# trailofbits/reverie

Measured on AMD Instinct MI355X. Metric: prover AND-gates/sec on GF(2) Bristol circuit; 1/2/4/8-GPU; proof bit-exact, higher is better.
Workload: dtype u32; 1 GPU; synthetic layered AND/XOR GF(2) circuit, 10027008 gates (5014185 AND), 4096 inputs, 153 layers x 65536, p_and=0.5, 256 reps x 8 players, 40 online; parallelism=reps/1, levels=163, compile_hint=RV_COMPILE_WHOLE_PROVER, gate_stream_bytes=334698564

## Files before the change

reverie_amd/csrc/interp.hip:

```cpp
#include <stdlib.h>

#include <algorithm>

#include "gf2dev.h"
#include "internal.h"
#include "launch.h"

namespace rv {

static size_t g_device_lds_limit = 160 * 1024;
void set_device_lds_limit(size_t bytes) { g_device_lds_limit = bytes; }
size_t device_lds_limit() { return g_device_lds_limit; }


__device__ __forceinline__ uint32_t gather_rows(const uint32_t* rows, const uint32_t* ids, uint32_t NQ, uint32_t q) {
    uint32_t v = 0;
#pragma unroll
    for (int i = 0; i < RV_LIN_K; i++) v ^= rows[(size_t)ids[i] * NQ + q];
    return v;
}
__device__ __forceinline__ uint32_t gather_corr_byte(const uint8_t* corr, const uint32_t* ids, uint32_t NQ, uint32_t o) {
    uint32_t v = 0;
#pragma unroll
    for (int i = 0; i < RV_LIN_K; i++) v ^= corr[(size_t)ids[i] * (NQ >> 1) + o];
    return v;
}
__device__ __forceinline__ uint32_t gather_corr(const uint8_t* corr, const uint32_t* ids, uint32_t NQ, uint32_t q) {
    return (gather_corr_byte(corr, ids, NQ, q >> 1) >> (4 * (q & 1))) & 0xFu;
}

__device__ __forceinline__ uint32_t gather_vclr(const uint8_t* vclr, const uint32_t* ids) {
    uint32_t v = 0;
#pragma unroll
    for (int i = 0; i < RV_LIN_K; i++) v ^= vclr[ids[i]];
    return v;
}

__device__ __forceinline__ uint32_t vc_nib(uint64_t c, uint32_t q) {
    const uint32_t w = (q & 8) ? (uint32_t)(c >> 32) : (uint32_t)c;
    return q < 16 ? (w >> (4 * (q & 7))) & 0xFu : 0u;
}
__device__ __forceinline__ uint64_t gather_vc(const uint64_t* vc, const uint32_t* ids) {
    uint64_t v = 0;
#pragma unroll
    for (int i = 0; i < RV_LIN_K; i++) v ^= vc[ids[i]];
    return v;
}
__device__ __forceinline__ void vc_store(uint64_t* vc, size_t row, uint32_t q, uint32_t smeared) {
    uint32_t v = q < 16 ? compress4(smeared) << (4 * (q & 7)) : 0u;
    v |= (uint32_t)__builtin_amdgcn_update_dpp(0, (int)v, 0x111, 0xF, 0xF, true);
    v |= (uint32_t)__builtin_amdgcn_update_dpp(0, (int)v, 0x112, 0xF, 0xF, true);
    v |= (uint32_t)__builtin_amdgcn_update_dpp(0, (int)v, 0x114, 0xF, 0xF, true);
    if (q == 7 || q == 15) ((uint32_t*)(vc + row))[q >> 3] = v;
}
constexpr bool is_verify(int mode) { return mode == MODE_VERIFY || mode == MODE_VERIFY_C; }

template <int MODE>
__device__ __forceinline__ void interp_one(const Gate& g, const InterpParams& p, uint32_t NQ, uint32_t q, uint32_t onm) {
    switch (g_op(g)) {
    case G_INPUT: {
        const uint32_t lam = p.rows[(size_t)g.m * NQ + q];
        uint32_t corr;
        if (!is_verify(MODE)) {
            const uint32_t w = p.wit[g.x] ? 0xFFFFFFFFu : 0u;
            corr = w ^ recon32(lam);
        } else {
            corr = onm ? (p.sup_in[(size_t)g.x * p.sup_nq + q] & onm) : 0u;
        }
        if (!is_verify(MODE) || onm) p.on[(size_t)g.eo * NQ + q] = corr;
        if (MODE == MODE_PROVE_V) {
            if (q == 0) p.vclr[g.dst] = p.wit[g.x] ? 1 : 0;
        } else if (MODE == MODE_VERIFY_C) {
            vc_store(p.vc, g.dst, q, corr);
        } else {
            store_bits(p.corr, g.dst, NQ, q, corr);
        }
        break;
    }
    case G_XORK: {
        p.rows[(size_t)g.dst * NQ + q] = gather_rows(p.rows, g.a, NQ, q) ^ gather_rows(p.rows, g.b, NQ, q);
        if (MODE == MODE_PROVE_V) {
            if (q == 0) p.vclr[g.dst] = (uint8_t)((g_ca(g) ^ gather_vclr(p.vclr, g.a) ^ gather_vclr(p.vclr, g.b)) & 1u);
            break;
        }
        if (MODE == MODE_VERIFY_C) {
            if (q == 0) p.vc[g.dst] = gather_vc(p.vc, g.a) ^ gather_vc(p.vc, g.b) ^ (g_ca(g) ? ~0ull : 0ull);
            break;
        }
        if (!(q & 1)) {
            const size_t h = NQ >> 1, o = q >> 1;
            const uint32_t c = (g_ca(g) ? 0xFFu : 0u) ^ gather_corr_byte(p.corr, g.a, NQ, o) ^ gather_corr_byte(p.corr, g.b, NQ, o);
            p.corr[(size_t)g.dst * h + o] = (uint8_t)c;
        }
        break;
    }
    case G_RANDOM: {
        if (MODE == MODE_VERIFY_C) {
            if (q == 0) p.vc[g.dst] = 0;
            break;
        }
        if (!(q & 1)) p.corr[(size_t)g.dst * (NQ >> 1) + (q >> 1)] = 0;
        break;
    }
    case G_MUL: {
        const uint32_t lx = gather_rows(p.rows, g.a, NQ, q), ly = gather_rows(p.rows, g.b, NQ, q);
        const uint32_t lab = p.rows[(size_t)g.m * NQ + q], lnew = p.rows[(size_t)(g.m + 1) * NQ + q];
        const uint32_t a = recon32(lx), b = recon32(ly), c = recon32(lab);
        uint32_t cx, cy, vx = 0, vy = 0;
        if (MODE == MODE_PROVE_V) {
            vx = (gather_vclr(p.vclr, g.a) ^ g_ca(g)) & 1u;
            vy = (gather_vclr(p.vclr, g.b) ^ g_cb(g)) & 1u;
            cx = a ^ (vx ? 0xFFFFFFFFu : 0u);
            cy = b ^ (vy ? 0xFFFFFFFFu : 0u);
        } else if (MODE == MODE_VERIFY_C) {
            cx = expand4(vc_nib(gather_vc(p.vc, g.a), q)) ^ (g_ca(g) ? 0xFFFFFFFFu : 0u);
            cy = expand4(vc_nib(gather_vc(p.vc, g.b), q)) ^ (g_cb(g) ? 0xFFFFFFFFu : 0u);
        } else {
            cx = expand4(gather_corr(p.corr, g.a, NQ, q)) ^ (g_ca(g) ? 0xFFFFFFFFu : 0u);
            cy = expand4(gather_corr(p.corr, g.b, NQ, q)) ^ (g_cb(g) ? 0xFFFFFFFFu : 0u);
        }
        uint32_t delta = (a & b) ^ c;
        uint32_t s = (ly & cx) ^ (lx & cy) ^ lab ^ lnew;
        uint32_t r;
        if (!is_verify(MODE)) {
            r = recon32(s);
        } else {
            if (onm) {
                delta = (p.sup_corr[(size_t)g.ep * p.sup_nq + q] & onm) | (delta & ~onm);
                s ^= p.sup_rec[(size_t)g.x * p.sup_nq + q];
            }
            r = recon32(s) & onm;
        }
        if (!is_verify(MODE) || onm) p.on[(size_t)g.eo * NQ + q] = s;
        store_bits(p.pre, g.ep, NQ, q, delta);
        if (MODE == MODE_PROVE_V) {
            if (q == 0) p.vclr[g.dst] = (uint8_t)(vx & vy);
        } else if (MODE == MODE_VERIFY_C) {
            vc_store(p.vc, g.dst, q, r ^ delta ^ (cx & cy));
        } else {
            store_bits(p.corr, g.dst, NQ, q, r ^ delta ^ (cx & cy));
        }
        break;
    }
    case G_RECON: {
        uint32_t m = gather_rows(p.rows, g.a, NQ, q);
        if (is_verify(MODE) && onm) m ^= p.sup_rec[(size_t)g.x * p.sup_nq + q];
        if (MODE == MODE_PROVE || onm) p.on[(size_t)g.eo * NQ + q] = m;
        uint32_t r = recon32(m);
        if (is_verify(MODE)) r &= onm;
        const uint32_t cx = expand4(gather_corr(p.corr, g.a, NQ, q)) ^ (g_ca(g) ? 0xFFFFFFFFu : 0u);
        p.rows[(size_t)g.dst * NQ + q] = 0;
        store_bits(p.corr, g.dst, NQ, q, r ^ cx);
        break;
    }
    case G_ASSERT: {
        uint32_t m = gather_rows(p.rows, g.a, NQ, q);
        if (is_verify(MODE) && onm) m ^= p.sup_rec[(size_t)g.x * p.sup_nq + q];
        if (!is_verify(MODE) || onm) p.on[(size_t)g.eo * NQ + q] = m;
        if (MODE == MODE_PROVE_V) {
            if (q == 0 && ((gather_vclr(p.vclr, g.a) ^ g_ca(g)) & 1u) != 0) atomicOr(p.err, RV_E_WITNESS_INVALID);
        } else {
            const uint32_t cx = expand4(MODE == MODE_VERIFY_C ? vc_nib(gather_vc(p.vc, g.a), q) : gather_corr(p.corr, g.a, NQ, q)) ^ (g_ca(g) ? 0xFFFFFFFFu : 0u);
            if (MODE == MODE_PROVE) {
                if ((recon32(m) ^ cx) != 0) atomicOr(p.err, RV_E_WITNESS_INVALID);
            } else {
                if (((recon32(m) ^ cx) & onm) != 0) atomicOr(p.err, RV_DEV_ZERO_CHECK);
            }
        }
        break;
    }
    default:
        break;
    }
}

template <int MODE>
__global__ __launch_bounds__(256) void k_interp(const Gate* __restrict__ gates, uint32_t lo, uint32_t hi, InterpParams p) {
    const uint32_t NQ = p.NQ;
    const uint32_t tid = blockIdx.x * blockDim.x + threadIdx.x;
    const uint32_t q = tid % NQ;
    const uint32_t worker = tid / NQ;
    const uint32_t n_workers = (gridDim.x * blockDim.x) / NQ;
    const uint32_t onm = (is_verify(MODE)) ? p.on_mask[q] : 0u;
    for (uint32_t gi = lo + worker; gi < hi; gi += n_workers) {
        const Gate g = gates[gi];
        interp_one<MODE>(g, p, NQ, q, onm);
    }
}

#ifndef RV_INTERP_UNROLL
#define RV_INTERP_UNROLL 4
#endif
#ifndef RV_INTERP_UNROLL_SMALL
#define RV_INTERP_UNROLL_SMALL 2
#endif
#ifndef RV_INTERP_UNROLL_MID
#define RV_INTERP_UNROLL_MID 4
#endif
#ifndef RV_INTERP_UNROLL_FAST
#define RV_INTERP_UNROLL_FAST 4
#endif
#ifndef RV_INTERP_UXOR_FAST
#define RV_INTERP_UXOR_FAST 0
#endif
__host__ __device__ constexpr int interp_unroll(int NQ, bool general = true) {
    return NQ >= 64 ? (general ? RV_INTERP_UNROLL : RV_INTERP_UNROLL_FAST) : NQ >= 32 ? RV_INTERP_UNROLL_MID : RV_INTERP_UNROLL_SMALL;
}

struct PfPlan {
    uint32_t dist;
    uint32_t rem;
    uint32_t n[2][4];
    uint32_t start[2][4];
};
template <uint32_t STEP>
__device__ __forceinline__ const Gate* pf_target(const Gate* __restrict__ gates, const PfPlan& pf, uint32_t t) {
    uint32_t tt = t + pf.dist;
#pragma unroll
    for (int k = 0; k < 2; k++) {
#pragma unroll
        for (int c = 0; c < 4; c++) {
            if (tt < pf.n[k][c]) return gates + pf.start[k][c] + tt * STEP;
            tt -= pf.n[k][c];
        }
        tt += pf.rem;
    }
    return nullptr;
}
template <uint32_t STEP>
__device__ __forceinline__ uint32_t pf_touch(const Gate* g, uint32_t lane) {
    constexpr uint32_t BYTES = STEP * (uint32_t)sizeof(Gate), NL = (BYTES + 127) / 128;
    uint32_t v = 0;
    if (g && lane <= NL) v = *(const uint32_t*)((const char*)g + (lane < NL ? lane * 128 : BYTES - 4));
    return v;
}
__device__ __forceinline__ void pf_sink(uint32_t v) { asm volatile("" ::"v"(v)); }

template <int MODE, int NQ, int U, int KA, int KB>
__device__ __forceinline__ void mulU(const Gate* __restrict__ gates, uint32_t g0, const InterpParams& p, uint32_t sub, uint32_t q,
                                     uint32_t onm, const Gate* pf = nullptr) {
    constexpr uint32_t GPW = 64 / NQ, H = NQ / 2;
    const bool on_wr = !is_verify(MODE) || ((__ballot(onm != 0) >> ((sub * NQ + q) & ~7u)) & 0xFFull) != 0;
    Gate g[U];
#pragma unroll
    for (int u = 0; u < U; u++) g[u] = gates[g0 + u * GPW + sub];
    uint32_t lx[U], ly[U], lab[U], lnew[U], bx[U], by[U], sc[U], sr[U];
    uint32_t ra[U][KA], ca[U][KA], rb[U][KB], cb[U][KB];
    const uint32_t* const vc32 = (const uint32_t*)p.vc + ((q >> 3) & 1u);
#pragma unroll
    for (int u = 0; u < U; u++) {
        const int na = (int)g_na(g[u]), nb = (int)g_nb(g[u]);
#pragma unroll
        for (int i = 0; i < KA; i++) {
            ra[u][i] = 0;
            ca[u][i] = 0;
            if (i == 0 || i < na) {
                ra[u][i] = p.rows[(size_t)g[u].a[i] * NQ + q];
                ca[u][i] = MODE == MODE_VERIFY_C ? vc32[2 * (size_t)g[u].a[i]]
                                                 : MODE == MODE_PROVE_V ? p.vclr[g[u].a[i]] : p.corr[(size_t)g[u].a[i] * H + (q >> 1)];
            }
        }
#pragma unroll
        for (int i = 0; i < KB; i++) {
            rb[u][i] = 0;
            cb[u][i] = 0;
            if (i == 0 || i < nb) {
                rb[u][i] = p.rows[(size_t)g[u].b[i] * NQ + q];
                cb[u][i] = MODE == MODE_VERIFY_C ? vc32[2 * (size_t)g[u].b[i]]
                                                 : MODE == MODE_PROVE_V ? p.vclr[g[u].b[i]] : p.corr[(size_t)g[u].b[i] * H + (q >> 1)];
            }
        }
        lab[u] = __builtin_nontemporal_load(&p.rows[(size_t)g[u].m * NQ + q]);
        lnew[u] = p.rows[(size_t)(g[u].m + 1) * NQ + q];
        if (is_verify(MODE)) {
            sc[u] = sr[u] = 0;
            if (onm) {
                sc[u] = p.sup_corr[(size_t)g[u].ep * p.sup_nq + q];
                sr[u] = p.sup_rec[(size_t)g[u].x * p.sup_nq + q];
            }
        }
    }
    const uint32_t pfv = pf_touch<U * GPW>(pf, sub * NQ + q);
#pragma unroll
    for (int u = 0; u < U; u++) {
        lx[u] = ra[u][0];
        bx[u] = ca[u][0];
        ly[u] = rb[u][0];
        by[u] = cb[u][0];
#pragma unroll
        for (int i = 1; i < KA; i++) {
            lx[u] ^= ra[u][i];
            bx[u] ^= ca[u][i];
        }
#pragma unroll
        for (int i = 1; i < KB; i++) {
            ly[u] ^= rb[u][i];
            by[u] ^= cb[u][i];
        }
    }
#pragma unroll
    for (int u = 0; u < U; u++) {
        const uint32_t a = recon32(lx[u]), b = recon32(ly[u]), c = recon32(lab[u]);
        uint32_t cx, cy;
        const uint32_t vx = (bx[u] ^ g_ca(g[u])) & 1u, vy = (by[u] ^ g_cb(g[u])) & 1u;
        if (MODE == MODE_PROVE_V) {
            cx = a ^ (vx ? 0xFFFFFFFFu : 0u);
            cy = b ^ (vy ? 0xFFFFFFFFu : 0u);
        } else if (MODE == MODE_VERIFY_C) {
            cx = expand4(q < 16 ? (bx[u] >> (4 * (q & 7))) & 0xFu : 0u) ^ (g_ca(g[u]) ? 0xFFFFFFFFu : 0u);
            cy = expand4(q < 16 ? (by[u] >> (4 * (q & 7))) & 0xFu : 0u) ^ (g_cb(g[u]) ? 0xFFFFFFFFu : 0u);
        } else {
            cx = expand4((bx[u] >> (4 * (q & 1))) & 0xFu) ^ (g_ca(g[u]) ? 0xFFFFFFFFu : 0u);
            cy = expand4((by[u] >> (4 * (q & 1))) & 0xFu) ^ (g_cb(g[u]) ? 0xFFFFFFFFu : 0u);
        }
        uint32_t delta = (a & b) ^ c;
        uint32_t s = (ly[u] & cx) ^ (lx[u] & cy) ^ lab[u] ^ lnew[u];
        uint32_t r = 0;
        if (MODE == MODE_PROVE) {
            r = recon32(s);
        } else if (is_verify(MODE)) {
            delta = (sc[u] & onm) | (delta & ~onm);
            s ^= sr[u];
            r = recon32(s) & onm;
        }
        if (!is_verify(MODE) || on_wr) __builtin_nontemporal_store(s, &p.on[(size_t)g[u].eo * NQ + q]);
        store_bits(p.pre, g[u].ep, NQ, q, delta);
        if (MODE == MODE_PROVE_V) {
            if (q == 0) p.vclr[g[u].dst] = (uint8_t)(vx & vy);
        } else if (MODE == MODE_VERIFY_C) {
            vc_store(p.vc, g[u].dst, q, r ^ delta ^ (cx & cy));
        } else {
            store_bits(p.corr, g[u].dst, NQ, q, r ^ delta ^ (cx & cy));
        }
    }
    pf_sink(pfv);
}

template <int MODE, int NQ, int U, int N>
__device__ __forceinline__ void xorU(const Gate* __restrict__ gates, uint32_t g0, const InterpParams& p, uint32_t sub, uint32_t q,
                                     const Gate* pf = nullptr) {
    constexpr uint32_t GPW = 64 / NQ, H = NQ / 2;
    Gate g[U];
#pragma unroll
    for (int u = 0; u < U; u++) g[u] = gates[g0 + u * GPW + sub];
    uint32_t x[U], bx[U], rr[U][N], cc[U][N];
#pragma unroll
    for (int u = 0; u < U; u++) {
        const int na = (int)g_na(g[u]), nb = (int)g_nb(g[u]);
#pragma unroll
        for (int i = 0; i < N; i++) {
            const uint32_t id = (N == 2) ? g[u].a[i] : (i < RV_LIN_K ? g[u].a[i] : g[u].b[i - RV_LIN_K]);
            rr[u][i] = 0;
            cc[u][i] = 0;
            if (N == 2 || (i < RV_LIN_K ? i < na : i - RV_LIN_K < nb)) {
                rr[u][i] = p.rows[(size_t)id * NQ + q];
                if (MODE == MODE_PROVE_V) {
                    if (q == 0) cc[u][i] = p.vclr[id];
                } else if (MODE == MODE_VERIFY_C) {
                    if (q < 2) cc[u][i] = ((const uint32_t*)p.vc)[2 * (size_t)id + q];
                } else if (q < H) {
                    cc[u][i] = p.corr[(size_t)id * H + q];
                }
            }
        }
    }
    const uint32_t pfv = pf_touch<U * GPW>(pf, sub * NQ + q);
#pragma unroll
    for (int u = 0; u < U; u++) {
        x[u] = 0;
        bx[u] = 0;
#pragma unroll
        for (int i = 0; i < N; i++) {
            x[u] ^= rr[u][i];
            bx[u] ^= cc[u][i];
        }
    }
#pragma unroll
    for (int u = 0; u < U; u++) {
        p.rows[(size_t)g[u].dst * NQ + q] = x[u];
        if (MODE == MODE_PROVE_V) {
            if (q == 0) p.vclr[g[u].dst] = (uint8_t)((bx[u] ^ g_ca(g[u])) & 1u);
        } else if (MODE == MODE_VERIFY_C) {
            if (q < 2) ((uint32_t*)p.vc)[2 * (size_t)g[u].dst + q] = bx[u] ^ (g_ca(g[u]) ? 0xFFFFFFFFu : 0u);
        } else if (q < H) {
            p.corr[(size_t)g[u].dst * H + q] = (uint8_t)(bx[u] ^ (g_ca(g[u]) ? 0xFFu : 0u));
        }
    }
    pf_sink(pfv);
}

template <int MODE, int NQ, bool GENERAL = true, bool PF = false, int UXOR = 0>
__device__ __forceinline__ void run_level(const Gate* __restrict__ gates, const LevelRange& r, const InterpParams& p, uint32_t wave,
                                          uint32_t n_waves, uint32_t lane, uint32_t onm, const Gate* pf_gates = nullptr,
                                          const PfPlan* pf = nullptr) {
    constexpr uint32_t GPW = 64 / NQ;
    const uint32_t q = lane % NQ, sub = lane / NQ;
    constexpr int U = interp_unroll(NQ, GENERAL);
    constexpr int UX = UXOR ? UXOR : U;
    static_assert(!PF || UX == U, "the prefetch plan assumes one step size");
    uint32_t slot = 0;
    auto my = [&](uint32_t used) { return (wave + n_waves - used % n_waves) % n_waves; };
    const uint32_t begin[5] = {r.lo, r.mul11, r.mul, r.xor2, r.xork}, end[5] = {r.mul11, r.mul, r.xor2, r.xork, r.hi};
    uint32_t rest[5];
#pragma unroll
    for (int c = 0; c < 4; c++) {
        const uint32_t STEP = (uint32_t)(c >= 2 ? UX : U) * GPW;
        const uint32_t n_full = (!GENERAL && (c == 1 || c == 3)) ? 0u : (end[c] - begin[c]) / STEP;
        rest[c] = begin[c] + n_full * STEP;
        for (uint32_t g0 = begin[c] + my(slot) * STEP; g0 < rest[c]; g0 += n_waves * STEP) {
            const Gate* t = nullptr;
            if (PF && pf->dist) t = pf_target<U * GPW>(pf_gates, *pf, slot + (g0 - begin[c]) / STEP);
            if (c == 0) mulU<MODE, NQ, U, 1, 1>(gates, g0, p, sub, q, onm, t);
            if (c == 1 && GENERAL) mulU<MODE, NQ, U, RV_LIN_K, RV_LIN_K>(gates, g0, p, sub, q, onm, t);
            if (c == 2) xorU<MODE, NQ, UX, 2>(gates, g0, p, sub, q, t);
            if (c == 3 && GENERAL) xorU<MODE, NQ, UX, 2 * RV_LIN_K>(gates, g0, p, sub, q, t);
        }
        slot += n_full;
    }
    rest[4] = begin[4];
    uint32_t cum[6];
    cum[0] = 0;
#pragma unroll
    for (int c = 0; c < 5; c++) cum[c + 1] = cum[c] + (end[c] - rest[c] + GPW - 1) / GPW;
    for (uint32_t t = my(slot); t < cum[5]; t += n_waves) {
        uint32_t c0 = rest[0], e0 = end[0], base = 0;
#pragma unroll
        for (int c = 1; c < 5; c++)
            if (t >= cum[c]) c0 = rest[c], e0 = end[c], base = cum[c];
        const uint32_t gi = c0 + (t - base) * GPW + sub;
        if (gi < e0) interp_one<MODE>(gates[gi], p, NQ, q, onm);
    }
}

template <int MODE, int NQ, bool GENERAL>
__global__ __launch_bounds__(256, MODE == MODE_VERIFY_C ? (GENERAL ? 4 : 7) : (GENERAL || NQ != 64) ? 1 : 8) void k_interp_full(const Gate* __restrict__ gates, LevelRange r, InterpParams p, PfPlan pf) {
    __builtin_amdgcn_s_setprio(1);
    const uint32_t lane = threadIdx.x & 63;
    const uint32_t wave = __builtin_amdgcn_readfirstlane((blockIdx.x * blockDim.x + threadIdx.x) >> 6);
    const uint32_t n_waves = gridDim.x * (blockDim.x >> 6);
    const uint32_t onm = (is_verify(MODE)) ? p.on_mask[lane % NQ] : 0u;
    constexpr int UXL = (!GENERAL && NQ == 64) ? RV_INTERP_UXOR_FAST : 0;
    constexpr bool PFL = UXL == 0 || UXL == interp_unroll(NQ, GENERAL);
    run_level<MODE, NQ, GENERAL, PFL, UXL>(gates, r, p, wave, n_waves, lane, onm, gates, &pf);
}

template <int MODE, int NQ>
__global__ __launch_bounds__(256) void k_interp_full_b(const Gate* __restrict__ gates, LevelRange r, const InterpParams* __restrict__ pp) {
    const InterpParams p = pp[blockIdx.y];
    const uint32_t lane = threadIdx.x & 63;
    const uint32_t wave = __builtin_amdgcn_readfirstlane((blockIdx.x * blockDim.x + threadIdx.x) >> 6);
    const uint32_t n_waves = gridDim.x * (blockDim.x >> 6);
    const uint32_t onm = (is_verify(MODE)) ? p.on_mask[lane % NQ] : 0u;
    run_level<MODE, NQ>(gates, r, p, wave, n_waves, lane, onm);
}

static bool level_is_general(const LevelRange& r) { return (r.mul - r.mul11) + (r.xork - r.xor2) >= 64; }

static uint32_t pf_dist(int NQ) {
    static const int env = [] {
        const char* e = getenv("RV_PF_DIST");
        return e ? atoi(e) : -1;
    }();
    const uint32_t v = env >= 0 ? (uint32_t)env : (NQ == 64 ? 4096u : 0u);
    return v & ~31u;
}

template <int NQ>
static PfPlan make_pf_plan(const LevelRange& r, const LevelRange* next) {
    constexpr uint32_t GPW = 64 / NQ;
    PfPlan pf{};
    pf.dist = pf_dist(NQ);
    if (!pf.dist) return pf;
    const LevelRange* lr[2] = {&r, next};
    uint32_t total = 0;
    for (int k = 0; k < 2; k++) {
        if (!lr[k]) break;
        const LevelRange& x = *lr[k];
        const bool general = level_is_general(x);
        const uint32_t step = (uint32_t)interp_unroll(NQ, general) * GPW;
        const uint32_t begin[4] = {x.lo, x.mul11, x.mul, x.xor2}, end[4] = {x.mul11, x.mul, x.xor2, x.xork};
        for (int c = 0; c < 4; c++) {
            pf.start[k][c] = begin[c];
            pf.n[k][c] = (!general && (c == 1 || c == 3)) ? 0u : (end[c] - begin[c]) / step;
            if (k == 0) total += pf.n[k][c];
        }
    }
    pf.rem = total & 31u;
    return pf;
}

template <int MODE, int NQ>
static void launch_interp_full_mode(hipStream_t st, dim3 grid, bool general, const Gate* d_gates, const LevelRange& r, const InterpParams& p,
                                    const PfPlan& pf) {
    if (general)
        hipLaunchKernelGGL((k_interp_full<MODE, NQ, true>), grid, dim3(256), 0, st, d_gates, r, p, pf);
    else
        hipLaunchKernelGGL((k_interp_full<MODE, NQ, false>), grid, dim3(256), 0, st, d_gates, r, p, pf);
}

template <int NQ>
static void launch_interp_full(hipStream_t st, int mode, const Gate* d_gates, const LevelRange& r, const InterpParams& p,
                               const LevelRange* next) {
    constexpr uint32_t GPW = 64 / NQ;
    const bool general = level_is_general(r);
    const PfPlan pf = make_pf_plan<NQ>(r, next);
    const uint32_t u = (uint32_t)interp_unroll(NQ, general);
    uint64_t waves = ((uint64_t)(r.hi - r.lo) + u * GPW - 1) / (u * GPW);
    uint64_t blocks = (waves + 3) / 4;
    if (blocks > 4096) blocks = 4096;
    if (blocks < 1) blocks = 1;
    const dim3 grid((unsigned)blocks);
    if (mode == MODE_PROVE_V) return launch_interp_full_mode<MODE_PROVE_V, NQ>(st, grid, general, d_gates, r, p, pf);
    if (mode == MODE_PROVE) return launch_interp_full_mode<MODE_PROVE, NQ>(st, grid, general, d_gates, r, p, pf);
    if constexpr (NQ == 64)
        if (mode == MODE_VERIFY_C) return launch_interp_full_mode<MODE_VERIFY_C, NQ>(st, grid, general, d_gates, r, p, pf);
    launch_interp_full_mode<MODE_VERIFY, NQ>(st, grid, general, d_gates, r, p, pf);
}


bool any_level_general(const LevelRange* lr, size_t n_levels) {
    for (size_t l = 0; l < n_levels; l++)
        if (level_is_general(lr[l])) return true;
    return false;
}

constexpr uint32_t NARROW_MAX_LEVELS = 1024;
constexpr uint32_t NARROW_WIN = 1024;
template <int MODE, int NQT, bool LEAN = false>
__device__ __forceinline__ void interp_narrow_body(const Gate* __restrict__ gates, const LevelRange* __restrict__ level_range,
                                                   uint32_t l0, uint32_t l1, const InterpParams& p) {
    __shared__ LevelRange s_lr[NARROW_MAX_LEVELS];
    __shared__ __attribute__((aligned(16))) Gate s_g[NARROW_WIN];
    const uint32_t NQ = NQT ? (uint32_t)NQT : p.NQ;
    const uint32_t lane = threadIdx.x & 63, wave = threadIdx.x >> 6;
    const uint32_t onm = (is_verify(MODE)) ? p.on_mask[NQT ? lane % NQ : threadIdx.x % NQ] : 0u;
    const uint32_t n_lv = l1 - l0;
    {
        const uint32_t* src = (const uint32_t*)(level_range + l0);
        uint32_t* dst = (uint32_t*)s_lr;
        for (uint32_t i = threadIdx.x; i < n_lv * (uint32_t)(sizeof(LevelRange) / 4); i += 1024) dst[i] = src[i];
    }
    __syncthreads();
    const uint32_t g_end = s_lr[n_lv - 1].hi;
    uint32_t win_lo = s_lr[0].lo, win_hi = win_lo;
    for (uint32_t l = 0; l < n_lv; l++) {
        const LevelRange r = s_lr[l];
        if (r.hi > win_hi) {
            win_lo = r.lo;
            win_hi = (r.lo + NARROW_WIN < g_end) ? r.lo + NARROW_WIN : g_end;
            const uint4* src = (const uint4*)(gates + win_lo);
            uint4* dst = (uint4*)s_g;
            for (uint32_t i = threadIdx.x; i < (win_hi - win_lo) * (uint32_t)(sizeof(Gate) / 16); i += 1024) dst[i] = src[i];
            __syncthreads();
        }
        const Gate* g = s_g - win_lo;
        if (NQT) {
            if (LEAN)
                run_level<MODE, NQT ? NQT : 64, false, false, 8>(g, r, p, wave, 16, lane, onm);
            else
                run_level<MODE, NQT ? NQT : 64>(g, r, p, wave, 16, lane, onm);
        } else {
            const uint32_t q = threadIdx.x % NQ, worker = threadIdx.x / NQ, n_workers = 1024 / NQ;
            for (uint32_t gi = r.lo + worker; gi < r.hi; gi += n_workers) interp_one<MODE>(g[gi], p, NQ, q, onm);
        }
        __syncthreads();
    }
}

template <int MODE, int NQT, bool LEAN = false>
__global__ __launch_bounds__(1024) void k_interp_narrow(const Gate* __restrict__ gates, const LevelRange* __restrict__ level_range,
                                                        uint32_t l0, uint32_t l1, InterpParams p) {
    interp_narrow_body<MODE, NQT, LEAN>(gates, level_range, l0, l1, p);
}
template <int MODE, int NQT>
__global__ __launch_bounds__(1024) void k_interp_narrow_b(const Gate* __restrict__ gates, const LevelRange* __restrict__ level_range,
                                                          uint32_t l0, uint32_t l1, const InterpParams* __restrict__ pp) {
    const InterpParams p = pp[blockIdx.x];
    interp_narrow_body<MODE, NQT>(gates, level_range, l0, l1, p);
}

template <int NQT, bool LEAN = false>
static void launch_narrow_nq(hipStream_t st, int mode, const Gate* d_gates, const LevelRange* d_lr, uint32_t a, uint32_t b,
                             const InterpParams& p) {
    if (mode == MODE_PROVE)
        hipLaunchKernelGGL((k_interp_narrow<MODE_PROVE, NQT, LEAN>), dim3(1), dim3(1024), 0, st, d_gates, d_lr, a, b, p);
    else
        hipLaunchKernelGGL((k_interp_narrow<MODE_VERIFY, NQT, LEAN>), dim3(1), dim3(1024), 0, st, d_gates, d_lr, a, b, p);
}

void launch_interp_narrow(hipStream_t st, int mode, const Gate* d_gates, const LevelRange* d_level_range, uint32_t l0, uint32_t l1,
                          int tiny, const InterpParams& p) {
    for (uint32_t a = l0; a < l1; a += NARROW_MAX_LEVELS) {
        const uint32_t b = (a + NARROW_MAX_LEVELS < l1) ? a + NARROW_MAX_LEVELS : l1;
        switch (tiny == 1 ? 0u : p.NQ) {
        case 64:
            if (tiny == 2)
                launch_narrow_nq<64, true>(st, mode, d_gates, d_level_range, a, b, p);
            else
                launch_narrow_nq<64>(st, mode, d_gates, d_level_range, a, b, p);
            break;
        case 32: launch_narrow_nq<32>(st, mode, d_gates, d_level_range, a, b, p); break;
        case 16: launch_narrow_nq<16>(st, mode, d_gates, d_level_range, a, b, p); break;
        case 8: launch_narrow_nq<8>(st, mode, d_gates, d_level_range, a, b, p); break;
        default: launch_narrow_nq<0>(st, mode, d_gates, d_level_range, a, b, p); break;
        }
    }
}

void launch_interp(hipStream_t st, int mode, const Gate* d_gates, const LevelRange& r, const InterpParams& p, const LevelRange* next) {
    if (r.hi <= r.lo) return;
    switch (p.NQ) {
    case 64: return launch_interp_full<64>(st, mode, d_gates, r, p, next);
    case 32: return launch_interp_full<32>(st, mode, d_gates, r, p, next);
    case 16: return launch_interp_full<16>(st, mode, d_gates, r, p, next);
    case 8: return launch_interp_full<8>(st, mode, d_gates, r, p, next);
    default: break;
    }
    const uint64_t want = (uint64_t)(r.hi - r.lo) * p.NQ;
    uint64_t blocks = (want + 255) / 256;
    if (blocks > 8192) blocks = 8192;
    if (mode == MODE_PROVE)
        hipLaunchKernelGGL(k_interp<MODE_PROVE>, dim3((unsigned)blocks), dim3(256), 0, st, d_gates, r.lo, r.hi, p);
    else
        hipLaunchKernelGGL(k_interp<MODE_VERIFY>, dim3((unsigned)blocks), dim3(256), 0, st, d_gates, r.lo, r.hi, p);
}

void launch_interp_batched(hipStream_t st, const Gate* d_gates, const LevelRange& r, const InterpParams* d_pp, uint32_t batch, int mode) {
    if (r.hi <= r.lo || !batch) return;
    uint64_t waves = ((uint64_t)(r.hi - r.lo) + RV_INTERP_UNROLL - 1) / RV_INTERP_UNROLL;
    uint64_t blocks = (waves + 3) / 4;
    const uint64_t cap = std::max<uint64_t>(4096 / batch, 1);
    if (blocks > cap) blocks = cap;
    if (mode == MODE_PROVE)
        hipLaunchKernelGGL((k_interp_full_b<MODE_PROVE, 64>), dim3((unsigned)blocks, batch), dim3(256), 0, st, d_gates, r, d_pp);
    else
        hipLaunchKernelGGL((k_interp_full_b<MODE_VERIFY, 64>), dim3((unsigned)blocks, batch), dim3(256), 0, st, d_gates, r, d_pp);
}

void launch_interp_narrow_batched(hipStream_t st, const Gate* d_gates, const LevelRange* d_level_range, uint32_t l0, uint32_t l1,
                                  int tiny, const InterpParams* d_pp, uint32_t batch, int mode) {
    for (uint32_t a = l0; a < l1 && batch; a += NARROW_MAX_LEVELS) {
        const uint32_t b = (a + NARROW_MAX_LEVELS < l1) ? a + NARROW_MAX_LEVELS : l1;
        if (mode == MODE_PROVE) {
            if (tiny == 1)
                hipLaunchKernelGGL((k_interp_narrow_b<MODE_PROVE, 0>), dim3(batch), dim3(1024), 0, st, d_gates, d_level_range, a, b, d_pp);
            else
                hipLaunchKernelGGL((k_interp_narrow_b<MODE_PROVE, 64>), dim3(batch), dim3(1024), 0, st, d_gates, d_level_range, a, b, d_pp);
        } else {
            if (tiny == 1)
                hipLaunchKernelGGL((k_interp_narrow_b<MODE_VERIFY, 0>), dim3(batch), dim3(1024), 0, st, d_gates, d_level_range, a, b, d_pp);
            else
                hipLaunchKernelGGL((k_interp_narrow_b<MODE_VERIFY, 64>), dim3(batch), dim3(1024), 0, st, d_gates, d_level_range, a, b, d_pp);
        }
    }
}

}
```

Measured before the change: 983.4 million AND gates/s.

## Spread PROVE_V clear-value byte loads across lanes and combine via ballot

In the PROVE_V path with NQ=64, the per-gate clear-value bytes (vclr) were loaded redundantly by every lane, or only by lane 0, as a chain of serial byte gathers. Each wave now assigns eight lanes per gate: six load the input ids' bytes and one holds the dst id. The bits are collected with a ballot, parities are computed by popcount, and one designated lane stores the result. This cuts redundant scalar-like byte loads and the q==0 divergent stores, at the cost of extra ballot and popcount work, a sched_barrier, and a constraint that U is at most 8.

```diff
diff --git a/reverie_amd/csrc/interp.hip b/reverie_amd/csrc/interp.hip
--- a/reverie_amd/csrc/interp.hip
+++ b/reverie_amd/csrc/interp.hip
@@ -1,3 +1,4 @@
+#include <stddef.h>
 #include <stdlib.h>
 
 #include <algorithm>
@@ -236,50 +237,91 @@
 }
 __device__ __forceinline__ void pf_sink(uint32_t v) { asm volatile("" ::"v"(v)); }
 
+constexpr bool vlane_path(int mode, int NQ) { return mode == MODE_PROVE_V && NQ == 64; }
+struct VLane {
+    uint32_t id;
+    bool out;
+};
+template <int U>
+__device__ __forceinline__ VLane vlane_ids(const Gate* g, uint32_t lane) {
+    constexpr uint32_t W = sizeof(Gate) / 4, WA = offsetof(Gate, a) / 4, WD = offsetof(Gate, dst) / 4;
+    static_assert(U <= 8 && 2 * RV_LIN_K <= 6 && offsetof(Gate, b) == offsetof(Gate, a) + 4 * RV_LIN_K, "a lane group of 8 per gate: six slots + dst");
+    const uint32_t u = lane >> 3, r = lane & 7;
+    VLane v;
+    v.out = u < U && r == 6;
+    v.id = ((const uint32_t*)g)[u < U && r < 7 ? u * W + (r == 6 ? WD : WA + r) : WA];
+    return v;
+}
+__device__ __forceinline__ uint32_t vlane_load(const uint8_t* vclr, const VLane& v) {
+    __builtin_amdgcn_sched_barrier(0);
+    return vclr[v.id];
+}
+__device__ __forceinline__ uint64_t vlane_bits(uint32_t b) { return __ballot((b & 1u) != 0); }
+__device__ __forceinline__ uint32_t vlane_parity(uint64_t bits, int u, uint32_t mask) {
+    return (uint32_t)__builtin_popcount((uint32_t)(bits >> (8 * u)) & mask) & 1u;
+}
+__device__ __forceinline__ void vlane_store(uint8_t* vclr, const VLane& v, uint32_t lane, uint32_t res) {
+    if (v.out) vclr[v.id] = (uint8_t)((res >> (lane >> 3)) & 1u);
+}
+
 template <int MODE, int NQ, int U, int KA, int KB>
 __device__ __forceinline__ void mulU(const Gate* __restrict__ gates, uint32_t g0, const InterpParams& p, uint32_t sub, uint32_t q,
                                      uint32_t onm, const Gate* pf = nullptr) {
     constexpr uint32_t GPW = 64 / NQ, H = NQ / 2;
     const bool on_wr = !is_verify(MODE) || ((__ballot(onm != 0) >> ((sub * NQ + q) & ~7u)) & 0xFFull) != 0;
+    constexpr bool VL = vlane_path(MODE, NQ);
     Gate g[U];
 #pragma unroll
     for (int u = 0; u < U; u++) g[u] = gates[g0 + u * GPW + sub];
+    VLane vl{};
+    if (VL) vl = vlane_ids<U>(gates + g0, q);
     uint32_t lx[U], ly[U], lab[U], lnew[U], bx[U], by[U], sc[U], sr[U];
     uint32_t ra[U][KA], ca[U][KA], rb[U][KB], cb[U][KB];
     const uint32_t* const vc32 = (const uint32_t*)p.vc + ((q >> 3) & 1u);
-#pragma unroll
-    for (int u = 0; u < U; u++) {
-        const int na = (int)g_na(g[u]), nb = (int)g_nb(g[u]);
-#pragma unroll
-        for (int i = 0; i < KA; i++) {
-            ra[u][i] = 0;
-            ca[u][i] = 0;
-            if (i == 0 || i < na) {
-                ra[u][i] = p.rows[(size_t)g[u].a[i] * NQ + q];
-                ca[u][i] = MODE == MODE_VERIFY_C ? vc32[2 * (size_t)g[u].a[i]]
-                                                 : MODE == MODE_PROVE_V ? p.vclr[g[u].a[i]] : p.corr[(size_t)g[u].a[i] * H + (q >> 1)];
+    constexpr int NPH = VL && (KA > 1 || KB > 1) ? 2 : 1;
+    uint32_t vv = 0;
+#pragma unroll
+    for (int ph = 0; ph < NPH; ph++) {
+        if (NPH == 2 && ph == 1) vv = vlane_load(p.vclr, vl);
+#pragma unroll
+        for (int u = 0; u < U; u++) {
+            const int na = (int)g_na(g[u]), nb = (int)g_nb(g[u]);
+#pragma unroll
+            for (int i = 0; i < KA; i++) {
+                if (NPH == 2 && (i == 0) != (ph == 0)) continue;
+                ra[u][i] = 0;
+                ca[u][i] = 0;
+                if (i == 0 || i < na) {
+                    ra[u][i] = p.rows[(size_t)g[u].a[i] * NQ + q];
+                    ca[u][i] = MODE == MODE_VERIFY_C ? vc32[2 * (size_t)g[u].a[i]]
+                                                     : MODE == MODE_PROVE_V ? (VL ? 0u : p.vclr[g[u].a[i]]) : p.corr[(size_t)g[u].a[i] * H + (q >> 1)];
+                }
             }
-        }
-#pragma unroll
-        for (int i = 0; i < KB; i++) {
-            rb[u][i] = 0;
-            cb[u][i] = 0;
-            if (i == 0 || i < nb) {
-                rb[u][i] = p.rows[(size_t)g[u].b[i] * NQ + q];
-                cb[u][i] = MODE == MODE_VERIFY_C ? vc32[2 * (size_t)g[u].b[i]]
-                                                 : MODE == MODE_PROVE_V ? p.vclr[g[u].b[i]] : p.corr[(size_t)g[u].b[i] * H + (q >> 1)];
+#pragma unroll
+            for (int i = 0; i < KB; i++) {
+                if (NPH == 2 && (i == 0) != (ph == 0)) continue;
+                rb[u][i] = 0;
+                cb[u][i] = 0;
+                if (i == 0 || i < nb) {
+                    rb[u][i] = p.rows[(size_t)g[u].b[i] * NQ + q];
+                    cb[u][i] = MODE == MODE_VERIFY_C ? vc32[2 * (size_t)g[u].b[i]]
+                                                     : MODE == MODE_PROVE_V ? (VL ? 0u : p.vclr[g[u].b[i]]) : p.corr[(size_t)g[u].b[i] * H + (q >> 1)];
+                }
             }
-        }
-        lab[u] = __builtin_nontemporal_load(&p.rows[(size_t)g[u].m * NQ + q]);
-        lnew[u] = p.rows[(size_t)(g[u].m + 1) * NQ + q];
-        if (is_verify(MODE)) {
-            sc[u] = sr[u] = 0;
-            if (onm) {
-                sc[u] = p.sup_corr[(size_t)g[u].ep * p.sup_nq + q];
-                sr[u] = p.sup_rec[(size_t)g[u].x * p.sup_nq + q];
+            if (ph != 0) continue;
+            lab[u] = __builtin_nontemporal_load(&p.rows[(size_t)g[u].m * NQ + q]);
+            lnew[u] = p.rows[(size_t)(g[u].m + 1) * NQ + q];
+            if (is_verify(MODE)) {
+                sc[u] = sr[u] = 0;
+                if (onm) {
+                    sc[u] = p.sup_corr[(size_t)g[u].ep * p.sup_nq + q];
+                    sr[u] = p.sup_rec[(size_t)g[u].x * p.sup_nq + q];
+                }
             }
         }
     }
+    if (VL && NPH == 1) vv = vlane_load(p.vclr, vl);
+    const uint64_t vbits = VL ? vlane_bits(vv) : 0;
     const uint32_t pfv = pf_touch<U * GPW>(pf, sub * NQ + q);
 #pragma unroll
     for (int u = 0; u < U; u++) {
@@ -298,11 +340,19 @@
             by[u] ^= cb[u][i];
         }
     }
+    uint32_t vres = 0;
 #pragma unroll
     for (int u = 0; u < U; u++) {
         const uint32_t a = recon32(lx[u]), b = recon32(ly[u]), c = recon32(lab[u]);
         uint32_t cx, cy;
-        const uint32_t vx = (bx[u] ^ g_ca(g[u])) & 1u, vy = (by[u] ^ g_cb(g[u])) & 1u;
+        uint32_t vx = (bx[u] ^ g_ca(g[u])) & 1u, vy = (by[u] ^ g_cb(g[u])) & 1u;
+        if (VL) {
+            constexpr uint32_t K = (1u << RV_LIN_K) - 1;
+            const uint32_t ma = KA == 1 ? 1u : (((1u << g_na(g[u])) - 1) & K) | 1u, mb = KB == 1 ? 1u : (((1u << g_nb(g[u])) - 1) & K) | 1u;
+            vx = vlane_parity(vbits, u, ma) ^ g_ca(g[u]);
+            vy = vlane_parity(vbits, u, mb << RV_LIN_K) ^ g_cb(g[u]);
+            vres |= (vx & vy) << u;
+        }
         if (MODE == MODE_PROVE_V) {
             cx = a ^ (vx ? 0xFFFFFFFFu : 0u);
             cy = b ^ (vy ? 0xFFFFFFFFu : 0u);
@@ -326,13 +376,14 @@
         if (!is_verify(MODE) || on_wr) __builtin_nontemporal_store(s, &p.on[(size_t)g[u].eo * NQ + q]);
         store_bits(p.pre, g[u].ep, NQ, q, delta);
         if (MODE == MODE_PROVE_V) {
-            if (q == 0) p.vclr[g[u].dst] = (uint8_t)(vx & vy);
+            if (!VL && q == 0) p.vclr[g[u].dst] = (uint8_t)(vx & vy);
         } else if (MODE == MODE_VERIFY_C) {
             vc_store(p.vc, g[u].dst, q, r ^ delta ^ (cx & cy));
         } else {
             store_bits(p.corr, g[u].dst, NQ, q, r ^ delta ^ (cx & cy));
         }
     }
+    if (VL) vlane_store(p.vclr, vl, q, vres);
     pf_sink(pfv);
 }
 
@@ -340,30 +391,42 @@
 __device__ __forceinline__ void xorU(const Gate* __restrict__ gates, uint32_t g0, const InterpParams& p, uint32_t sub, uint32_t q,
                                      const Gate* pf = nullptr) {
     constexpr uint32_t GPW = 64 / NQ, H = NQ / 2;
+    constexpr bool VL = vlane_path(MODE, NQ);
     Gate g[U];
 #pragma unroll
     for (int u = 0; u < U; u++) g[u] = gates[g0 + u * GPW + sub];
+    VLane vl{};
+    if (VL) vl = vlane_ids<U>(gates + g0, q);
     uint32_t x[U], bx[U], rr[U][N], cc[U][N];
-#pragma unroll
-    for (int u = 0; u < U; u++) {
-        const int na = (int)g_na(g[u]), nb = (int)g_nb(g[u]);
-#pragma unroll
-        for (int i = 0; i < N; i++) {
-            const uint32_t id = (N == 2) ? g[u].a[i] : (i < RV_LIN_K ? g[u].a[i] : g[u].b[i - RV_LIN_K]);
-            rr[u][i] = 0;
-            cc[u][i] = 0;
-            if (N == 2 || (i < RV_LIN_K ? i < na : i - RV_LIN_K < nb)) {
-                rr[u][i] = p.rows[(size_t)id * NQ + q];
-                if (MODE == MODE_PROVE_V) {
-                    if (q == 0) cc[u][i] = p.vclr[id];
-                } else if (MODE == MODE_VERIFY_C) {
-                    if (q < 2) cc[u][i] = ((const uint32_t*)p.vc)[2 * (size_t)id + q];
-                } else if (q < H) {
-                    cc[u][i] = p.corr[(size_t)id * H + q];
+    constexpr int NPH = VL && N > 2 ? 2 : 1;
+    uint32_t vv = 0;
+#pragma unroll
+    for (int ph = 0; ph < NPH; ph++) {
+        if (NPH == 2 && ph == 1) vv = vlane_load(p.vclr, vl);
+#pragma unroll
+        for (int u = 0; u < U; u++) {
+            const int na = (int)g_na(g[u]), nb = (int)g_nb(g[u]);
+#pragma unroll
+            for (int i = 0; i < N; i++) {
+                if (NPH == 2 && (i == 0) != (ph == 0)) continue;
+                const uint32_t id = (N == 2) ? g[u].a[i] : (i < RV_LIN_K ? g[u].a[i] : g[u].b[i - RV_LIN_K]);
+                rr[u][i] = 0;
+                cc[u][i] = 0;
+                if (N == 2 || (NPH == 2 && i == 0) || (i < RV_LIN_K ? i < na : i - RV_LIN_K < nb)) {
+                    rr[u][i] = p.rows[(size_t)id * NQ + q];
+                    if (MODE == MODE_PROVE_V) {
+                        if (!VL && q == 0) cc[u][i] = p.vclr[id];
+                    } else if (MODE == MODE_VERIFY_C) {
+                        if (q < 2) cc[u][i] = ((const uint32_t*)p.vc)[2 * (size_t)id + q];
+                    } else if (q < H) {
+                        cc[u][i] = p.corr[(size_t)id * H + q];
+                    }
                 }
             }
         }
     }
+    if (VL && NPH == 1) vv = vlane_load(p.vclr, vl);
+    const uint64_t vbits = VL ? vlane_bits(vv) : 0;
     const uint32_t pfv = pf_touch<U * GPW>(pf, sub * NQ + q);
 #pragma unroll
     for (int u = 0; u < U; u++) {
@@ -375,10 +438,15 @@
             bx[u] ^= cc[u][i];
         }
     }
+    uint32_t vres = 0;
 #pragma unroll
     for (int u = 0; u < U; u++) {
         p.rows[(size_t)g[u].dst * NQ + q] = x[u];
-        if (MODE == MODE_PROVE_V) {
+        if (VL) {
+            constexpr uint32_t K = (1u << RV_LIN_K) - 1;
+            const uint32_t m = N == 2 ? 3u : (((1u << g_na(g[u])) - 1) & K) | ((((1u << g_nb(g[u])) - 1) & K) << RV_LIN_K);
+            vres |= (vlane_parity(vbits, u, m) ^ g_ca(g[u])) << u;
+        } else if (MODE == MODE_PROVE_V) {
             if (q == 0) p.vclr[g[u].dst] = (uint8_t)((bx[u] ^ g_ca(g[u])) & 1u);
         } else if (MODE == MODE_VERIFY_C) {
             if (q < 2) ((uint32_t*)p.vc)[2 * (size_t)g[u].dst + q] = bx[u] ^ (g_ca(g[u]) ? 0xFFFFFFFFu : 0u);
@@ -386,6 +454,7 @@
             p.corr[(size_t)g[u].dst * H + q] = (uint8_t)(bx[u] ^ (g_ca(g[u]) ? 0xFFu : 0u));
         }
     }
+    if (VL) vlane_store(p.vclr, vl, q, vres);
     pf_sink(pfv);
 }
 
```

Result: slower. 968.7 million AND gates/s (-1.5%).
